# CSMaus/DefectDetection_viaObjectDetection

Measured on AMD Instinct MI355X. Metric: images/sec @640x640 b32 YOLOv8s-seg, higher is better.
Workload: dtype fp16

## Files before the change

defectdetection_viaobjectdetection_amd/_capi.py:

```python
from __future__ import annotations

import ctypes as C
import os

_HERE = os.path.dirname(os.path.abspath(__file__))
LIB_PATH = os.path.join(_HERE, "lib", "libmi355yolo.so")


class M355Error(RuntimeError):
    """Raised when a libmi355yolo call returns a negative status."""


class ModelDesc(C.Structure):
    _fields_ = [("scale", C.c_int), ("nc", C.c_int), ("in_h", C.c_int), ("in_w", C.c_int),
                ("max_batch", C.c_int)]


class ConvInfo(C.Structure):
    _fields_ = [("name", C.c_char * 64), ("cin", C.c_int), ("cout", C.c_int), ("k", C.c_int),
                ("stride", C.c_int), ("has_bn", C.c_int), ("transposed", C.c_int), ("act", C.c_int),
                ("groups", C.c_int)]


class OpInfo(C.Structure):
# ... 44 lines not shown


class LetterboxImage(C.Structure):
    _fields_ = [("offset", C.c_int64), ("h", C.c_int32), ("w", C.c_int32), ("uh", C.c_int32), ("uw", C.c_int32),
                ("top", C.c_int32), ("left", C.c_int32)]


_P = C.c_void_p
_F = C.POINTER(C.c_float)
SIGNATURES = {
    "m355_version": (C.c_char_p, []),
    "m355_last_error": (C.c_char_p, [_P]),
    "m355_create": (C.c_int, [C.POINTER(ModelDesc), C.POINTER(_P)]),
    "m355_destroy": (None, [_P]),
    "m355_num_convs": (C.c_int, [_P]),
    "m355_get_conv_info": (C.c_int, [_P, C.c_int, C.POINTER(ConvInfo)]),
    "m355_num_anchors": (C.c_int, [_P]),
    "m355_pred_width": (C.c_int, [_P]),
    "m355_proto_hw": (C.c_int, [_P, C.POINTER(C.c_int), C.POINTER(C.c_int)]),
    "m355_workspace_bytes": (C.c_size_t, [_P]),
    "m355_flops_per_image": (C.c_double, [_P]),
    "m355_set_conv_weights": (C.c_int, [_P, C.c_int, _P, _P]),
    "m355_forward": (C.c_int, [_P, _P, C.c_int, _P, _P, _P]),
    "m355_num_ops": (C.c_int, [_P]),
    "m355_get_op_info": (C.c_int, [_P, C.c_int, C.POINTER(OpInfo)]),
    "m355_set_profiling": (C.c_int, [_P, C.c_int]),
    "m355_collect_op_times": (C.c_int, [_P, C.POINTER(C.c_double), C.POINTER(C.c_long)]),
    "m355_get_raw_head": (C.c_int, [_P, C.POINTER(_P), C.POINTER(C.c_int)]),
    "m355_copy_raw_head": (C.c_int, [_P, C.c_int, _P, _P]),
    "m355_set_keep_raw": (C.c_int, [_P, C.c_int]),
    "m355_postprocess": (C.c_int, [_P, _P, _P, C.c_int, C.c_float, C.c_float, C.c_int, _P, _P, _P, _P]),
    "m355_conv2d_fwd": (C.c_int, [_P, C.c_int, C.c_int, C.c_int, C.c_int, _P, _P, C.c_int, C.c_int, C.c_int,
                                  C.c_int, _P, _P, C.c_int, C.c_int, _P]),
    "m355_c2f_c32_fwd": (C.c_int, [_P, C.c_int, C.c_int, C.c_int, _P, _P, _P, _P, _P, _P, C.c_int, _P, _P]),
    "m355_bneck_pair_fwd": (C.c_int, [_P, C.c_int, C.c_int, C.c_int, C.c_int, C.c_int, _P, _P, _P, _P, C.c_int, _P, C.c_int, _P]),
    "m355_s2c64_cv1_fwd": (C.c_int, [_P, C.c_int, C.c_int, C.c_int, _P, _P, _P, _P, _P, _P]),
    "m355_stem_s2c32_cv1_fwd": (C.c_int, [_P, C.c_int, C.c_int, C.c_int, _P, _P, _P, _P, _P, _P, _P, C.c_int, _P]),
    "m355_proto_phase_fwd": (C.c_int, [_P, C.c_int, C.c_int, C.c_int, _P, _P, _P, _P, _P, _P, _P, _P]),
    "m355_head_tail_fwd": (C.c_int, [_P, C.c_int, C.c_int, C.c_int, C.c_int, C.c_float, _P, _P, _P, _P, _P, _P, _P, C.c_int, C.c_int, _P]),
    "m355_tal_assign_launch": (C.c_int, [_P, _P, _P, _P, _P, _P, C.c_int32, C.c_int32, C.c_int32, C.c_int32, _P, _P, _P, _P, _P, _P]),
    "m355_conv2d_dgrad": (C.c_int, [_P, C.c_int, C.c_int, C.c_int, C.c_int, _P, C.c_int, C.c_int, C.c_int, _P, _P]),
    "m355_conv2d_wgrad": (C.c_int, [_P, _P, C.c_int, C.c_int, C.c_int, C.c_int, C.c_int, C.c_int, C.c_int, _P, _P]),
    "m355_bn_silu_train_fwd": (C.c_int, [_P, C.c_int, C.c_int, C.c_int, C.c_int, _P, _P, C.c_float, C.c_int, _P, _P, _P, _P, _P]),
    "m355_bn_silu_train_bwd": (C.c_int, [_P, _P, C.c_int, C.c_int, C.c_int, C.c_int, _P, _P, _P, _P, C.c_int, _P, _P, _P, _P]),
    "m355_bn_workspace_floats": (C.c_size_t, [C.c_int]),
    "m355_wgrad_workspace_bytes": (C.c_size_t, [C.c_int32, C.c_int32, C.c_int32, C.c_int32, C.c_int32, C.c_int32]),
    "m355_grad_sumsq_workspace_floats": (C.c_size_t, []),
    "m355_convt2x2_fwd": (C.c_int, [_P, C.c_int, C.c_int, C.c_int, C.c_int, _P, _P, C.c_int, _P, _P]),
    "m355_stem_fwd": (C.c_int, [_P, C.c_int, C.c_int, C.c_int, _P, _P, C.c_int, _P, _P]),
    "m355_stem6_fwd": (C.c_int, [_P, C.c_int, C.c_int, C.c_int, _P, _P, C.c_int, _P, _P]),
    "m355_dwconv3x3_fwd": (C.c_int, [_P, C.c_int, C.c_int, C.c_int, C.c_int, C.c_int, _P, _P, C.c_int, _P, C.c_int, _P]),
    "m355_psa_attn_fwd": (C.c_int, [_P, C.c_int, C.c_int, C.c_int, C.c_int, C.c_int, C.c_int, _P, _P, _P, _P]),
    "m355_sppf_pool": (C.c_int, [_P, C.c_int, C.c_int, C.c_int, C.c_int, _P, _P]),
    "m355_upsample2x": (C.c_int, [_P, C.c_int, C.c_int, C.c_int, C.c_int, _P, _P]),
    "m355_head_decode": (C.c_int, [_P, C.c_int, C.c_int, C.c_int, C.c_int, _P, _P]),
    "m355_nms": (C.c_int, [_P, C.c_int, C.c_int, C.c_int, C.c_int, C.c_float, C.c_float, C.c_int, _P, _P, _P]),
    "m355_conv_launch": (C.c_int, [C.POINTER(ConvLaunchArgs), _P]),
    "m355_wgrad_launch": (C.c_int, [C.POINTER(WgradLaunchArgs), _P]),
    "m355_bn_train_fwd_launch": (C.c_int, [_P, C.c_int64, C.c_int32, C.c_int32, _P, _P, C.c_float, C.c_int32, _P, C.c_int32,
                                           _P, C.c_int32, _P, _P, _P, _P, _P, C.c_float, _P]),
    "m355_bn_train_bwd_launch": (C.c_int, [_P, _P, C.c_int64, C.c_int32, C.c_int32, C.c_int32, _P, _P, _P, _P, C.c_int32,
                                           _P, C.c_int32, _P, _P, _P]),
    "m355_adamw_step": (C.c_int, [_P, _P, _P, _P, _P, _P, C.c_int64, C.c_float, C.c_float, C.c_float, C.c_float, C.c_float,
                                  C.c_float, C.c_int32, C.c_float, C.c_float, _P]),
    "m355_sgd_step": (C.c_int, [_P, _P, _P, _P, _P, C.c_int64, C.c_float, C.c_float, C.c_float, C.c_int32, C.c_float,
                                C.c_float, C.c_float, _P]),
# ... 71 lines not shown
```

defectdetection_viaobjectdetection_amd/csrc/conv1x1_wreg.hip:

```cpp
#include <stdio.h>
#include <stdlib.h>

#include <type_traits>

#include "common.h"

namespace m355 {
namespace {

typedef float float16v __attribute__((ext_vector_type(16)));
constexpr int NWAVES = 8;

__device__ __forceinline__ void dma16(__amdgpu_buffer_rsrc_t rsrc, int voff, int soff, char* lds) {
  __builtin_amdgcn_raw_ptr_buffer_load_lds(rsrc, (__attribute__((address_space(3))) void*)lds, 16, voff, soff, 0, 0);
}
__device__ __forceinline__ int row_plain(int rho) { return 16 * ((rho >> 2) & 1) + 4 * (rho >> 3) + (rho & 3); }

__device__ __forceinline__ void silu16(float16v& v) {
#pragma clang fp contract(off)
  float16v t;
#pragma unroll
  for (int j = 0; j < 16; ++j) t[j] = v[j] * -1.4426950408889634f;
#pragma unroll
  for (int j = 0; j < 16; ++j) t[j] = __builtin_amdgcn_exp2f(t[j]);
// ... 215 lines not shown
    }
    vb += nwg;
    ct = nct; p0 = np0;
    nct = nnct; np0 = nnp0;
    have1 = have2;
    if (ct != ct_cur) {
      load_weights(ct);
      __builtin_amdgcn_s_waitcnt(0x0070);
      __builtin_amdgcn_s_barrier();
    }
  }
}

template <int K, int CB, int PB = 2, bool SPLIT = false>
int launch_w1(const ConvArgs& a, hipStream_t s) {
  using C = W1<K, CB, PB>;
  const int ntiles_px = (a.M + C::TP - 1) / C::TP, ctiles = a.Cout / (CB * 32);
  const int ntiles = ntiles_px * ctiles;
  static int slots = 0;
  auto k = conv1x1_wreg_kernel<K, CB, PB, SPLIT>;
  if (!slots) {
    hipError_t e = hipFuncSetAttribute((const void*)k, hipFuncAttributeMaxDynamicSharedMemorySize, C::LDS_BYTES);
    if (e != hipSuccess) return (int)e;
    int dev = 0, cus = 0;
    if (hipGetDevice(&dev) != hipSuccess || hipDeviceGetAttribute(&cus, hipDeviceAttributeMultiprocessorCount, dev) != hipSuccess)
      return -2;
    slots = cus < 8 ? 8 : cus;
  }
  const int grid = ntiles <= slots ? ntiles : slots;
  hipLaunchKernelGGL(k, dim3(grid), dim3(64 * NWAVES), C::LDS_BYTES, s, a, ntiles_px, ntiles);
  return (int)hipGetLastError();
}

}

bool conv1x1_wreg_ok(const ConvArgs& a) {
  if (a.ksize != 1 || a.stride != 1 || a.pad != 0 || a.out_f32 || a.convt_co > 0 || a.tmode || a.phase || a.w2 || a.dec_preds ||
      a.res)
    return false;
  if (a.Cin != 128 && a.Cin != 192 && a.Cin != 256 && a.Cin != 384 && a.Cin != 512) return false;
  if (a.Cout % 128 || a.Cout > 512 || a.ldx % 8 || a.ldy % 8 || a.Kpad < a.Cin || a.Kpad % 8) return false;
  if (a.Ho != a.Hi || a.Wo != a.Wi) return false;
  if (a.x_bstride != (long)a.Hi * a.Wi * a.ldx || a.y_bstride != (long)a.Ho * a.Wo * a.ldy) return false;
  const int cb = a.Cout % 256 == 0 ? 8 : 4;
  if (cb == 4 && a.Cin > 384) return false;
  if (a.csplit > 0) {
    if (!(a.Cin == 384 && cb == 4) || !a.x2 || a.csplit != 256 || a.ldx2 % 8 || a.x2_bstride % 8 || (a.Hi & 1) ||
        (a.Wi & 1) || a.M >= (1 << 24) || a.M % ((long)a.Ho * a.Wo))
      return false;
    if ((a.M / ((long)a.Ho * a.Wo)) * a.x2_bstride * 2 >= (1L << 31)) return false;
  }
  return (long)a.M * a.ldx * 2 < (1L << 31) && (long)a.M * a.ldy < (1L << 31);
}

int launch_conv1x1_wreg(const ConvArgs& a, hipStream_t s) {
  if (!conv1x1_wreg_ok(a) || !conv_rows_covered(a, 128)) return -1;
  const bool c8 = a.Cout % 256 == 0;
  if (a.csplit > 0 && !(a.Cin == 384 && !c8)) return -1;
  switch (a.Cin) {
    case 128: return c8 ? launch_w1<128, 8>(a, s) : launch_w1<128, 4>(a, s);
    case 192: return c8 ? launch_w1<192, 8>(a, s) : launch_w1<192, 4>(a, s);
    case 256: return c8 ? launch_w1<256, 8>(a, s) : launch_w1<256, 4>(a, s);
    case 384: return c8 ? launch_w1<384, 8>(a, s) : (a.csplit > 0 ? launch_w1<384, 4, 1, true>(a, s) : launch_w1<384, 4, 1, false>(a, s));
    case 512: return c8 ? launch_w1<512, 8>(a, s) : -1;
  }
  return -1;
}

}
```

defectdetection_viaobjectdetection_amd/csrc/engine.hip:

```cpp
#include <math.h>
#include <stdio.h>
#include <stdlib.h>
#include <string.h>

#include <string>
#include <vector>

#include "../../include/mi355yolo.h"
#include "common.h"
#include "engine_types.h"
#include "switches.h"
#include "weight_pack.h"

using namespace m355;

thread_local std::string m355::g_err;

namespace {

void fuse_conv_cv1(m355_engine* e) {
  if (e->sw.no_cvfuse) return;
  for (size_t i = 0; i < e->ops.size(); ++i) {
    Op& oi = e->ops[i];
    if (oi.kind != OP_CONV || oi.out_ext != 0 || oi.res.t >= 0 || oi.in2.t >= 0) continue;
// ... 260 lines not shown
  const PhysConv& p = e->phys[op.conv];
  const Tensor& ti = e->tensors[op.in.t];
  HeadTailArgs a{};
  a.x = ti.p; a.ldx = ti.C; a.M = (long)B * ti.H * ti.W; a.HW = ti.H * ti.W; a.W = ti.W;
  a.stride = (float)(e->desc.in_h / ti.H);
  a.A = e->A; a.level_off = op.level_off; a.nc = e->nc; a.nm = e->nm;
  a.wf = p.wf; a.bias = p.bias; a.preds = preds;
  return a;
}

bool head_tail_layout(const m355_engine* e, const PhysConv& p) {
  return p.diag && p.logical.size() == 3 && p.cin == 224 && p.cout == 64 + e->nc + e->nm && e->nm == 32 && e->nc <= 32 &&
         e->convs[p.logical[0]].cin == 64 && e->convs[p.logical[1]].cin == 128;
}

void plan_route(m355_engine* e, Op& op, const ConvArgs& a) {
  const PlanSwitches& sw = e->sw;
  PhysConv& p = e->phys[op.conv];
  const Tensor& ti = e->tensors[op.in.t];
  if (op.kind == OP_PHASE) {
    op.tile = p.cout % 128 == 0 ? TILE_128x128 : TILE_64x128;
    if (p.l3 >= 0 && p.cin == 128 && p.cout == 128 && p.cout2 == 32 && ti.H % 8 == 0 && ti.W % 16 == 0 && !sw.no_protor)
      op.route = R_PROTOR;
    return;
  }
  const bool conv = op.kind == OP_CONV;
  op.tile = conv_pick_tile(a.Cout, a.M);
  if (a.ksize == 1 && op.tile == TILE_128x128 && sw.k1_tile >= 0) op.tile = sw.k1_tile;
  if (op.decode) op.tile = TILE_128x128;
  if (conv && conv3x3_halo_ok(a) && !sw.no_halo) op.route = R_HALO;
  const bool m32 = op.route == R_HALO && conv3x3_halo_pick(a, proc_switches().no_wide, proc_switches().no_m32) == TILE_M32;
  if (conv && conv3x3_c32_ok(a) && !sw.no_c32) op.route = R_C32;
  if (conv && op.out_ext == 0 && p.l3 < 0 && !p.diag && op.res.t < 0 && !op.decode && (op.in2.t < 0 || !sw.no_w1_split) &&
      conv1x1_wreg_ok(a) && !sw.no_w1)
    op.route = R_W1;
  if (conv && op.route != R_HALO && op.route != R_C32 && conv3x3_slab_ok(a) && !sw.no_slab) op.route = R_SLAB;
  const bool planes_s2 = p.k == 3 && p.stride == 2 && op.res.t < 0 && op.in2.t < 0 && !sw.no_planes_s2;
  const bool planes_m64 = m32 && a.Cout <= 64 && op.res.t < 0 && op.in2.t < 0 && !sw.no_planes_m64;
  if (conv && (op.route == R_SLAB || planes_s2 || planes_m64) && op.out_ext == 0 && p.l3 < 0 && !p.diag && !sw.no_planes) {
    PlanesArgs pa = planes_args(e, op, e->desc.max_batch, 0);
    pa.wfb = (const half_t*)1;
    if (conv3x3_planes_ok(pa)) {
      op.route = R_PLANES;
      p.planes = 1;
    }
  }
  if (conv && op.out_ext == 1 && !op.decode && head_tail_layout(e, p) && ti.C == 224 && op.in.off == 0 && op.raw_off == 0 &&
      a.Ho * a.Wo >= 32 && !sw.no_headtail) {
    op.headtail = 1;
    ++e->headtail_n;
  }
  if (conv && p.l3 >= 0 && p.k == 3 && p.stride == 2 && p.cin == 32 && p.cout == 64 && p.cout2 == 64 && a.Ho % 8 == 0 &&
      a.Wo % 16 == 0 && !sw.no_s2c32)
    op.route = R_S2C32;
  if (conv && p.l3 >= 0 && p.k == 3 && p.stride == 2 && p.cin == 64 && p.cout == 128 && p.cout2 == 128 && a.Ho % 8 == 0 &&
      a.Wo % 8 == 0 && !sw.no_s2c64)
    op.route = R_S2C64;
}

void conv_label(const m355_engine* e, Op& op, const ConvArgs& a) {
  static const char* tile_names[] = {"128x128", "64x128", "32x256", "64x256"};
  const PhysConv& p = e->phys[op.conv];
  char* k = op.kernel;
  const size_t n = sizeof(op.kernel);
  const char* ch = a.Cout > 64 ? "128ch" : "64ch";
  switch (op.route) {
    case R_IGEMM:
// ... 695 lines not shown
```

defectdetection_viaobjectdetection_amd/csrc/op_entries.hip:

```cpp
#include <math.h>
#include <stdio.h>
#include <stdlib.h>

#include <string>
#include <vector>

#include "../../include/mi355yolo.h"
#include "common.h"
#include "switches.h"
#include "weight_pack.h"

using namespace m355;

namespace {

int set_err(int code, const std::string& m) {
  g_err = m;
  return code;
}

struct DevBuf {
  std::vector<void*> p;
  ~DevBuf() { for (void* q : p) (void)hipFree(q); }
  void* alloc(size_t bytes) {
// ... 110 lines not shown
  if (force_tile >= 0 && (force_tile & 0xff) == TILE_PLANES) {
    PlanesArgs pa{};
    pa.x = a.x; pa.x_bstride = a.x_bstride; pa.ldx = a.ldx; pa.H = H; pa.W = W; pa.B = B; pa.Cin = cin; pa.Cout = cout; pa.stride = stride;
    pa.wfb = d.put(planes_frag_pack_padded(rows.data(), cout, Kpad, cin)); pa.cblocks_b = planes_cblocks(cout); pa.bb = a.bias;
    pa.y = (half_t*)d_y; pa.y_bstride = a.y_bstride; pa.ldy = a.ldy;
    pa.res = a.res; pa.r_bstride = a.r_bstride; pa.ldr = a.ldr; pa.act = act; pa.stamps = a.stamps;
    if (!pa.wfb) return alloc_failed();
    char what[80];
    snprintf(what, sizeof(what), "conv3x3_planes B=%d %dx%d %d->%d", B, H, W, cin, cout);
    rc = diag.reps(conv3x3_planes_ok(pa) ? launch_conv3x3_planes(pa, s) : -1, s, what, [&] { return launch_conv3x3_planes(pa, s); });
  } else
  for (int rep = 0; rep < (a.dbg ? 5 : 1); ++rep)
    rc = (force_tile >= 0 && (force_tile & 0xff) == TILE_W1) ? launch_conv1x1_wreg(a, s)
         : (force_tile >= 0 && (force_tile & 0xff) == TILE_C32)
             ? launch_conv3x3_c32(a, s)
             : ((force_tile >= 0 && (force_tile & 0xff) >= TILE_HALO) ? launch_conv3x3_halo(a, (force_tile & 0xff) - TILE_HALO, s)
                                                                       : launch_conv_igemm(a, force_tile, s));
  const hipError_t se = hipStreamSynchronize(s);
  diag.dump(se == hipSuccess);
  return launch_status(rc, se, "conv");
}

}

extern "C" {

int m355_conv2d_fwd(const void* d_x, int B, int H, int W, int cin, const float* h_w, const float* h_bias, int cout,
                    int k, int stride, int act, const void* d_res, void* d_y, int out_f32, int force_tile,
                    void* stream) {
  return conv_op_common(d_x, B, H, W, cin, h_w, h_bias, cout, k, stride, act, d_res, d_y, out_f32, force_tile, 0,
                        stream);
}

int m355_c2f_c32_fwd(const void* d_x, int B, int H, int W, const float* h_wa, const float* h_ba, const float* h_wb,
                     const float* h_bb, const float* h_wc, const float* h_bc, int shortcut, void* d_y, void* stream) {
  if (!d_x || !d_y || !h_wa || !h_ba || !h_wb || !h_bb || !h_wc || !h_bc) return set_err(M355_ERR_INVALID, "null pointer");
  if (B <= 0 || H <= 0 || W <= 0 || H % 8 || W % 16) return set_err(M355_ERR_INVALID, "H must be a multiple of 8 and W of 16");
  hipStream_t s = (hipStream_t)stream;
  const int kp3 = conv_kpad(32, 3), kp1 = conv_kpad(96, 1);
  std::vector<half_t> ra((size_t)32 * kp3, (half_t)0.f), rb((size_t)32 * kp3, (half_t)0.f), rc_((size_t)64 * kp1, (half_t)0.f);
  pack_conv_rows(h_wa, 32, 32, 3, kp3, 0, ra);
  pack_conv_rows(h_wb, 32, 32, 3, kp3, 0, rb);
  pack_conv_rows(h_wc, 64, 96, 1, kp1, 0, rc_);
  std::vector<float> bias(128);
  for (int i = 0; i < 32; ++i) { bias[i] = h_ba[i]; bias[32 + i] = h_bb[i]; }
  for (int i = 0; i < 64; ++i) bias[64 + i] = h_bc[i];
  const FragList fl = frag_list(3, 32, 32);
  DevBuf d;
  const float* db = d.put(bias);
  C2fC32Args a{};
  a.x = (const half_t*)d_x; a.x_bstride = (long)H * W * 64; a.ldx = 64; a.H = H; a.W = W; a.B = B;
  a.wa = d.put(ra); a.wb = d.put(rb); a.wc = d.put(rc_); a.kpad_a = kp3; a.kpad_b = kp3; a.kpad_c = kp1;
  a.waf = d.put(frag_pack(ra.data(), kp3, fl, false)); a.wbf = d.put(frag_pack(rb.data(), kp3, fl, true));
  if (!db || !a.wa || !a.wb || !a.wc || !a.waf || !a.wbf) return alloc_failed();
  a.ba = db; a.bb = db + 32; a.bc = db + 64;
  a.y = (half_t*)d_y; a.y_bstride = (long)H * W * 64; a.ldy = 64; a.shortcut = shortcut;
  const int rc = launch_c2f_c32(a, s);
  return launch_status(rc, hipStreamSynchronize(s), "c2f_c32");
}

int m355_bneck_pair_fwd(const void* d_x, int B, int H, int W, int C, int ldx, const float* h_wa, const float* h_ba, const float* h_wb,
                        const float* h_bb, int shortcut, void* d_y, int ldy, void* stream) {
  if (!d_x || !d_y || !h_wa || !h_ba || !h_wb || !h_bb) return set_err(M355_ERR_INVALID, "null pointer");
  if (B <= 0 || H <= 0 || W <= 0 || C <= 0 || ldx < C || ldy < C) return set_err(M355_ERR_INVALID, "bad shape");
  hipStream_t s = (hipStream_t)stream;
  if (C % 32) return set_err(M355_ERR_INVALID, "C must be a multiple of 32");
// ... 382 lines not shown
                     int mw, int in_h, int in_w, uint8_t* d_masks, void* stream) {
  if (!d_dets || !d_counts || !d_protos || !d_masks) return set_err(M355_ERR_INVALID, "null pointer");
  const int rc = launch_proto_masks(d_dets, d_counts, (const half_t*)d_protos, B, max_det, 32, mh, mw, in_h, in_w,
                                    d_masks, (hipStream_t)stream);
  return rc == 0 ? M355_OK : set_err(M355_ERR_HIP, "mask launch failed: " + std::to_string(rc));
}

int m355_conv_launch(const m355_conv_args* c, void* stream) {
  if (!c || !c->x || !c->w_packed || !c->bias || !c->y || !c->zero_page) return set_err(M355_ERR_INVALID, "null pointer");
  ConvArgs a{};
  a.x = (const half_t*)c->x; a.x_bstride = c->x_bstride; a.ldx = c->ldx; a.Hi = c->hi; a.Wi = c->wi; a.Cin = c->cin;
  a.w = (const half_t*)c->w_packed; a.Kpad = c->kpad; a.bias = c->bias;
  a.y = c->y; a.y_bstride = c->y_bstride; a.ldy = c->ldy; a.Ho = c->ho; a.Wo = c->wo; a.Cout = c->cout;
  a.res = (const half_t*)c->res; a.r_bstride = c->r_bstride; a.ldr = c->ldr;
  a.ksize = c->ksize; a.stride = c->stride; a.pad = c->pad; a.M = c->batch * c->ho * c->wo;
  a.act = c->act; a.out_f32 = c->out_f32; a.convt_co = c->convt_co; a.tmode = c->tmode;
  a.zero = (const half_t*)c->zero_page;
  if (c->convt_co > 0 && c->tmode == 0 && c->ksize == 1 && c->res)
    return set_err(M355_ERR_INVALID, "ConvTranspose (convt_co > 0, ksize 1) takes no residual");
  if (c->tmode == 2) {
    a.tmode = 0;
    a.phase = dgrad_phase_form(c->convt_co, c->cin, c->res != nullptr);
    if (!a.phase)
      return set_err(M355_ERR_INVALID, "tmode 2 needs convt_co % 64 == 0, or 128 % convt_co == 0 with convt_co >= 16 and no res "
                                       "(use the tmode 1 gather)");
  }
  int rc;
  const bool train_w1 = !proc_switches().no_train_w1;
  const bool train_c32 = !proc_switches().no_train_c32;
  if (a.phase == 2 && dgrad_s2c32_ok(a))
    rc = launch_dgrad_s2c32(a, (hipStream_t)stream);
  else if (!a.tmode && conv3x3_halo_ok(a))
    rc = launch_conv3x3_halo(a, 0, (hipStream_t)stream);
  else if (train_w1 && !a.tmode && conv1x1_wreg_ok(a))
    rc = launch_conv1x1_wreg(a, (hipStream_t)stream);
  else if (train_c32 && !a.tmode && conv3x3_c32_ok(a) && conv_rows_covered(a, 32))
    rc = launch_conv3x3_c32(a, (hipStream_t)stream);
  else
    rc = launch_conv_igemm(a, TILE_AUTO, (hipStream_t)stream);
  return rc == 0 ? M355_OK : set_err(M355_ERR_HIP, "conv launch failed: " + std::to_string(rc));
}

int m355_wgrad_launch(const m355_wgrad_args* w, void* stream) {
  if (!w || !w->dz || !w->x || !w->dw || !w->zero_page) return set_err(M355_ERR_INVALID, "null pointer");
  const int rc = launch_conv_wgrad((const half_t*)w->dz, w->dz_bstride, w->lddz, (const half_t*)w->x, w->x_bstride, w->ldx,
                                   w->batch, w->hi, w->wi, w->cin, w->ho, w->wo, w->cout, w->ksize, w->stride, w->pad,
                                   w->dw, (const half_t*)w->zero_page, w->ws, (size_t)(w->ws_bytes < 0 ? 0 : w->ws_bytes),
                                   (hipStream_t)stream);
  if (rc == -3) return set_err(M355_ERR_INVALID, "wgrad workspace missing or smaller than m355_wgrad_workspace_bytes()");
  return rc == 0 ? M355_OK : set_err(M355_ERR_HIP, "wgrad launch failed: " + std::to_string(rc));
}

int m355_bn_train_fwd_launch(const void* z, int64_t npix, int32_t ldz, int32_t C, const float* gamma, const float* beta,
                             float eps, int32_t act, void* y, int32_t ldy, const void* res, int32_t ldr, float* mean,
                             float* invstd, float* ws, float* running_mean, float* running_var, float momentum,
                             void* stream) {
  if (!z || !gamma || !beta || !y || !mean || !invstd || !ws) return set_err(M355_ERR_INVALID, "null pointer");
  const int rc = launch_bn_silu_train_fwd((const half_t*)z, npix, ldz, C, gamma, beta, eps, (half_t*)y, ldy,
                                          (const half_t*)res, ldr, ws, mean, invstd, act, running_mean, running_var, momentum,
                                          (hipStream_t)stream);
  return rc == 0 ? M355_OK : set_err(M355_ERR_HIP, "bn fwd launch failed: " + std::to_string(rc));
}

int m355_bn_train_bwd_launch(const void* z, const void* dy, int64_t npix, int32_t ldz, int32_t lddy, int32_t C,
                             const float* mean, const float* invstd, const float* gamma, const float* beta, int32_t act,
                             void* dz, int32_t lddz, float* dbeta_dgamma, float* ws, void* stream) {
  if (!z || !dy || !mean || !invstd || !gamma || !beta || !dz || !dbeta_dgamma || !ws) return set_err(M355_ERR_INVALID, "null pointer");
// ... 211 lines not shown
```

defectdetection_viaobjectdetection_amd/csrc/switches.h:

```cpp
#pragma once

namespace m355 {

struct ProcSwitches {
  bool no_fast_epi, no_wide, no_m32, no_bias_lds, static_tiles, no_persist, stem_gather;
  int persist, halo_variant, smallm;
  bool c2f_noprio;
  const char* c2f_stamps;
  int c32_waste, c32_slots, m32_slots, wide_slots, wide_stagger;
  int s2c32_dbg, s2c32_ring, s2c64_prio, protor_prio;
  const char *s2c32_stamps, *s2c64_stamps, *protor_stamps;
  int stem2_nxb;
  bool no_stemfuse;
  int sppf_minblocks, mask_dbg, mask_tile;
  bool no_dgrad_s2c32, no_wgrad_stem, no_wgrad_s2c32, no_wgrad3, no_train_w1, no_train_c32;
  int wgrad_blocks, w2_blocks_x2, wgrad3_shrink, wgrad3_blocks, wgrad3_mintiles;
  long wgrad3_slabmb;
};
const ProcSwitches& proc_switches();

struct PlanSwitches {
  bool no_c2f32, no_pair, no_protofuse, no_protofuse3, no_upfuse;
  int lane_plan[4];
  bool no_cvfuse, decfuse, no_lanes, no_subbatch;
  bool no_stemfuse;
  int subbatch, subbatch_ops;
  bool no_protor, no_halo, no_c32, no_w1_split, no_w1, no_slab, no_planes_s2, no_planes_m64, no_planes, no_headtail, no_s2c32,
      no_s2c64;
  int k1_tile;
  long headtail_maxm;
};
PlanSwitches read_plan_switches();

bool live_no_stem2();
bool live_no_dgrad_phases();
bool live_pair64();
const char* live_stamps_path();
int live_bneck_reps();

}
```

defectdetection_viaobjectdetection_amd/csrc/switches.hip:

```cpp
#include "switches.h"

#include <limits.h>
#include <stdlib.h>

namespace m355 {

namespace {

bool env_set(const char* name) { return getenv(name) != nullptr; }
long env_int(const char* name, long unset) {
  const char* v = getenv(name);
  return v ? atol(v) : unset;
}

ProcSwitches read_proc_switches() {
  ProcSwitches v{};
  v.no_fast_epi = env_set("M355_NO_FAST_EPI");
  v.no_wide = env_set("M355_NO_WIDE");
  v.no_m32 = env_set("M355_NO_M32");
  v.no_bias_lds = env_set("M355_NO_BIAS_LDS");
  v.static_tiles = env_set("M355_STATIC_TILES");
  v.no_persist = env_set("M355_NO_PERSIST");
  v.stem_gather = env_set("M355_STEM_GATHER");
  v.persist = env_int("M355_PERSIST", 0);
// ... 34 lines not shown
}

}

const ProcSwitches& proc_switches() {
  static const ProcSwitches v = read_proc_switches();
  return v;
}

PlanSwitches read_plan_switches() {
  PlanSwitches v{};
  v.no_c2f32 = env_set("M355_NO_C2F32");
  v.no_pair = env_set("M355_NO_PAIR");
  v.no_protofuse = env_set("M355_NO_PROTOFUSE");
  v.no_protofuse3 = env_set("M355_NO_PROTOFUSE3");
  v.no_upfuse = env_set("M355_NO_UPFUSE");
  const int lanes[4] = {1, 2, 2, 0};
  const char* lp = getenv("M355_LANE_PLAN");
  for (int i = 0; i < 4; ++i) {
    if (lp && (lp[i] < '0' || lp[i] > '3')) lp = nullptr;
    v.lane_plan[i] = lp ? lp[i] - '0' : lanes[i];
  }
  v.no_cvfuse = env_set("M355_NO_CVFUSE");
  v.decfuse = env_set("M355_DECFUSE");
  v.no_lanes = env_set("M355_NO_LANES");
  v.no_subbatch = env_set("M355_NO_SUBBATCH");
  v.no_stemfuse = env_set("M355_NO_STEMFUSE");
  v.subbatch = env_int("M355_SUBBATCH", 0);
  v.subbatch_ops = env_int("M355_SUBBATCH_OPS", INT_MAX);
  v.no_protor = env_set("M355_NO_PROTOR");
  v.no_halo = env_set("M355_NO_HALO");
  v.no_c32 = env_set("M355_NO_C32");
  v.no_w1_split = env_set("M355_NO_W1_SPLIT");
  v.no_w1 = env_set("M355_NO_W1");
  v.no_slab = env_set("M355_NO_SLAB");
  v.no_planes_s2 = env_set("M355_NO_PLANES_S2");
  v.no_planes_m64 = env_set("M355_NO_PLANES_M64");
  v.no_planes = env_set("M355_NO_PLANES");
  v.no_headtail = env_set("M355_NO_HEADTAIL");
  v.no_s2c32 = env_set("M355_NO_S2C32");
  v.no_s2c64 = env_set("M355_NO_S2C64");
  v.k1_tile = env_int("M355_K1_TILE", -1);
  v.headtail_maxm = env_int("M355_HEADTAIL_MAXM", 0);
  return v;
}

bool live_no_stem2() { return env_set("M355_NO_STEM2"); }
bool live_no_dgrad_phases() { return env_set("M355_NO_DGRAD_PHASES"); }
bool live_pair64() { return env_set("M355_PAIR64"); }
const char* live_stamps_path() { return getenv("M355_STAMPS"); }
int live_bneck_reps() { return env_int("M355_BNECK_REPS", 0); }

}
```

defectdetection_viaobjectdetection_amd/csrc/weight_pack.hip:

```cpp
#include "weight_pack.h"

#include <algorithm>

namespace m355 {

void pack_conv_rows(const float* w, int cout, int cin, int k, int Kpad, int row0, std::vector<half_t>& dst, int koff) {
  for (int co = 0; co < cout; ++co)
    for (int ci = 0; ci < cin; ++ci)
      for (int kh = 0; kh < k; ++kh)
        for (int kw = 0; kw < k; ++kw)
          dst[(size_t)(row0 + co) * Kpad + koff + (kh * k + kw) * cin + ci] =
              (half_t)w[(((size_t)co * cin + ci) * k + kh) * k + kw];
}

void pack_convt2x2_rows(const float* w, int cin, int cout, int Kpad, std::vector<half_t>& dst) {
  for (int c = 0; c < cin; ++c)
    for (int co = 0; co < cout; ++co)
      for (int dy = 0; dy < 2; ++dy)
        for (int dx = 0; dx < 2; ++dx)
          dst[(size_t)((dy * 2 + dx) * cout + co) * Kpad + c] = (half_t)w[(((size_t)c * cout + co) * 2 + dy) * 2 + dx];
}

std::vector<half_t> pack_stem3x3(const float* w, int cout) {
  std::vector<half_t> sw((size_t)cout * 32, (half_t)0.f);
// ... 4 lines not shown
  return sw;
}

std::vector<half_t> to_half_vec(const float* w, size_t n) {
  std::vector<half_t> r(n);
  for (size_t i = 0; i < n; ++i) r[i] = (half_t)w[i];
  return r;
}

static int frag_row(int rho, bool operand) {
  if (!operand) return 16 * ((rho >> 2) & 1) + 4 * (rho >> 3) + (rho & 3);
  const int q = rho >> 3, h = (rho >> 2) & 1, i = rho & 3;
  return 16 * (q >> 1) + 8 * h + 4 * (q & 1) + i;
}
std::vector<half_t> frag_pack(const half_t* rows, int Kpad, const FragList& frags, bool operand) {
  std::vector<half_t> out(frags.size() * 512);
  for (size_t f = 0; f < frags.size(); ++f)
    for (int lane = 0; lane < 64; ++lane) {
      const half_t* src = rows + (size_t)(frags[f].first + frag_row(lane & 31, operand)) * Kpad + frags[f].second + 8 * (lane >> 5);
      for (int j = 0; j < 8; ++j) out[(f * 64 + lane) * 8 + j] = src[j];
    }
  return out;
}
FragList frag_grid(int rows, int K) {
  FragList f;
  for (int r = 0; r < rows; r += 32)
    for (int k = 0; k < K; k += 16) f.push_back({r, k});
  return f;
}

FragList frag_list(int k, int cin, int cout) {
  const bool taken = (k == 3 && cin == 64 && cout == 128) ||
                     (k == 3 && cin == 32 && (cout == 64 || cout == 32)) ||
                     (k == 1 && (cin == 128 || cin == 192 || cin == 256 || cin == 384 || cin == 512) && cout % 128 == 0 && cout <= 512);
  return taken ? frag_grid(cout, k * k * cin) : FragList();
}

FragList head_level_frags(int nc) {
  FragList f = frag_grid(64, 64);
  for (int sl = 0; sl < 8; ++sl) f.push_back({64, 64 + 16 * sl});
  for (int sl = 0; sl < 2; ++sl) f.push_back({64 + nc, 192 + 16 * sl});
  return f;
}

FragList epilogue_frags(int cout2, int k) { return frag_grid(cout2, k); }

void compose_proto_phases(int n, const float* wtp, const float* btp, const float* w3p, const float* b3p, int cout_pad, int Kpad,
                          std::vector<half_t>& rows, std::vector<float>& btab) {
    rows.assign((size_t)cout_pad * Kpad, (half_t)0.f);
    std::vector<double> acc((size_t)n * n);
    for (int py = 0; py < 2; ++py)
      for (int px = 0; px < 2; ++px)
        for (int aa = 0; aa < 2; ++aa)
          for (int bb = 0; bb < 2; ++bb) {
            std::fill(acc.begin(), acc.end(), 0.0);
            for (int kh = 0; kh < 3; ++kh) {
              const int ty = py + kh - 1, ry = (ty < 0 ? -1 : ty / 2), dy = ty & 1;
              if (ry + 1 - py != aa) continue;
              for (int kw = 0; kw < 3; ++kw) {
                const int tx = px + kw - 1, rx = (tx < 0 ? -1 : tx / 2), dx = tx & 1;
                if (rx + 1 - px != bb) continue;
                for (int co = 0; co < n; ++co)
                  for (int c = 0; c < n; ++c) {
                    const double w3 = w3p[(((size_t)co * n + c) * 3 + kh) * 3 + kw];
                    if (w3 == 0.0) continue;
                    const float* wt = wtp;
                    double* ar = &acc[(size_t)co * n];
// ... 43 lines not shown
```

include/mi355yolo.h:

```cpp
#ifndef MI355YOLO_H_
#define MI355YOLO_H_

#include <stddef.h>
#include <stdint.h>

#ifdef __cplusplus
extern "C" {
#endif

typedef struct m355_engine m355_engine;

typedef enum {
  M355_OK = 0,
  M355_ERR_INVALID = -1,
  M355_ERR_NO_DEVICE = -2,
  M355_ERR_HIP = -3,
  M355_ERR_STATE = -4,
  M355_ERR_NOMEM = -5
} m355_status;

typedef struct {
  int scale;
  int nc;
  int in_h, in_w;
// ... 28 lines not shown
int m355_set_conv_weights(m355_engine* e, int idx, const float* w, const float* bias);

int m355_forward(m355_engine* e, const void* d_in_u8_nhwc, int batch, float* d_preds, void* d_protos,
                 void* stream);

typedef struct {
  char kernel[48];
  char layer[64];
  double flops_per_image;
  double bytes_per_image;
  double weight_bytes;
} m355_op_info;
int m355_num_ops(const m355_engine* e);
int m355_get_op_info(const m355_engine* e, int idx, m355_op_info* out);
int m355_set_profiling(m355_engine* e, int enable);
int m355_collect_op_times(m355_engine* e, double* ms_sum, long* counts);

int m355_get_raw_head(m355_engine* e, const float** d_raw, int* width);
int m355_copy_raw_head(m355_engine* e, int batch, float* d_out, void* stream);
int m355_set_keep_raw(m355_engine* e, int keep);

int m355_postprocess(m355_engine* e, const float* d_preds, const void* d_protos, int batch, float conf,
                     float iou, int max_det, float* d_dets, int* d_counts, uint8_t* d_masks, void* stream);
int m355_postprocess_ex(m355_engine* e, const float* d_preds, const void* d_protos, int batch, float conf, float iou,
                        int max_det, int agnostic, const uint32_t* d_class_mask, float* d_dets, int* d_counts,
                        uint8_t* d_masks, void* stream);



int m355_conv2d_fwd(const void* d_x_f16_nhwc, int B, int H, int W, int cin, const float* h_w,
                    const float* h_bias, int cout, int k, int stride, int act,
                    const void* d_res_f16_nhwc, void* d_y_f16_nhwc, int out_f32, int force_tile,
                    void* stream);
int m355_c2f_c32_fwd(const void* d_x_f16_nhwc, int B, int H, int W, const float* h_wa, const float* h_ba,
                     const float* h_wb, const float* h_bb, const float* h_wc, const float* h_bc, int shortcut,
                     void* d_y_f16_nhwc, void* stream);
int m355_bneck_pair_fwd(const void* d_x_f16_nhwc, int B, int H, int W, int C, int ldx, const float* h_wa, const float* h_ba,
                        const float* h_wb, const float* h_bb, int shortcut, void* d_y_f16_nhwc, int ldy, void* stream);
int m355_s2c64_cv1_fwd(const void* d_x_f16_nhwc, int B, int H, int W, const float* h_w3, const float* h_b3, const float* h_w1,
                       const float* h_b1, void* d_y_f16_nhwc, void* stream);
int m355_stem_s2c32_cv1_fwd(const void* d_in_u8_nhwc, int B, int H, int W, const float* h_w0, const float* h_b0, const float* h_w1,
                            const float* h_b1, const float* h_w2, const float* h_b2, void* d_y_f16_nhwc, int two_team, void* stream);
int m355_proto_phase_fwd(const void* d_x_f16_nhwc, int B, int H, int W, const float* h_wt, const float* h_bt, const float* h_w3,
                         const float* h_b3, const float* h_wc, const float* h_bc, void* d_y_f16_nhwc, void* stream);
int m355_head_tail_fwd(const void* d_x_f16_nhwc, int B, int H, int W, int nc, float stride, const float* h_w2, const float* h_b2,
                       const float* h_w3, const float* h_b3, const float* h_w4, const float* h_b4, float* d_preds, int A, int level_off,
                       void* stream);
int m355_conv2d_dgrad(const void* d_dy_f16_nhwc, int B, int H, int W, int cin, const float* h_w, int cout, int k,
                      int stride, void* d_dx_f16_nhwc, void* stream);
int m355_conv2d_wgrad(const void* d_x_f16_nhwc, const void* d_dy_f16_nhwc, int B, int H, int W, int cin, int cout,
                      int k, int stride, float* d_dw_krsc, void* stream);
size_t m355_bn_workspace_floats(int C);
int m355_bn_silu_train_fwd(const void* d_z, int B, int H, int W, int C, const float* d_gamma, const float* d_beta,
                           float eps, int act, void* d_y, float* d_mean, float* d_invstd, float* d_ws, void* stream);
int m355_bn_silu_train_bwd(const void* d_z, const void* d_dy, int B, int H, int W, int C, const float* d_mean,
                           const float* d_invstd, const float* d_gamma, const float* d_beta, int act, void* d_dz,
                           float* d_dbeta_dgamma, float* d_ws, void* stream);
int m355_convt2x2_fwd(const void* d_x_f16_nhwc, int B, int H, int W, int cin, const float* h_w,
                      const float* h_bias, int cout, void* d_y_f16_nhwc, void* stream);
int m355_stem_fwd(const void* d_in_u8, int B, int H, int W, const float* h_w, const float* h_bias, int cout,
                  void* d_y_f16_nhwc, void* stream);
int m355_stem6_fwd(const void* d_x_u8_nhwc, int B, int H, int W, const float* h_w, const float* h_bias, int C0,
                   void* d_y_f16_nhwc, void* stream);
int m355_dwconv3x3_fwd(const void* d_x_f16_nhwc, int B, int H, int W, int C, int ldx, const float* h_w, const float* h_b,
                       int act, void* d_y_f16_nhwc, int ldy, void* stream);
int m355_psa_attn_fwd(const void* d_qkv_f16_nhwc, int B, int H, int W, int heads, int key_dim, int head_dim,
// ... 171 lines not shown
```

Measured before the change: 18160.

## Add deep-K 1x1 conv kernel for Cin 768/1024 with weight-register streaming

Adds a new 1x1 convolution kernel for Cin of 768 and 1024 with Cout a multiple of 256. It streams activation tiles into an 8-stage LDS ring through buffer-to-LDS DMA and double-buffers weight chunks in registers, one 128-channel K chunk at a time. It also supports the concat-split input form, where the upsampled operand is read at half resolution from a second tensor. The engine routes these layers (for example the SPPF and neck C2f cv2 convs) to the new kernel by default; an env switch disables it, and training keeps the old path. A standalone conv_op test entry point is added as well.

```diff
diff --git a/defectdetection_viaobjectdetection_amd/_capi.py b/defectdetection_viaobjectdetection_amd/_capi.py
--- a/defectdetection_viaobjectdetection_amd/_capi.py
+++ b/defectdetection_viaobjectdetection_amd/_capi.py
@@ -100,6 +100,8 @@
     "m355_postprocess": (C.c_int, [_P, _P, _P, C.c_int, C.c_float, C.c_float, C.c_int, _P, _P, _P, _P]),
     "m355_conv2d_fwd": (C.c_int, [_P, C.c_int, C.c_int, C.c_int, C.c_int, _P, _P, C.c_int, C.c_int, C.c_int,
                                   C.c_int, _P, _P, C.c_int, C.c_int, _P]),
+    "m355_conv_op": (C.c_int, [_P, C.c_int, _P, C.c_int, C.c_int, C.c_int, C.c_int, C.c_int, C.c_int, _P, _P, C.c_int, C.c_int, _P,
+                               C.c_int, C.c_int, _P]),
     "m355_c2f_c32_fwd": (C.c_int, [_P, C.c_int, C.c_int, C.c_int, _P, _P, _P, _P, _P, _P, C.c_int, _P, _P]),
     "m355_bneck_pair_fwd": (C.c_int, [_P, C.c_int, C.c_int, C.c_int, C.c_int, C.c_int, _P, _P, _P, _P, C.c_int, _P, C.c_int, _P]),
     "m355_s2c64_cv1_fwd": (C.c_int, [_P, C.c_int, C.c_int, C.c_int, _P, _P, _P, _P, _P, _P]),
diff --git a/defectdetection_viaobjectdetection_amd/csrc/conv1x1_wreg.hip b/defectdetection_viaobjectdetection_amd/csrc/conv1x1_wreg.hip
--- a/defectdetection_viaobjectdetection_amd/csrc/conv1x1_wreg.hip
+++ b/defectdetection_viaobjectdetection_amd/csrc/conv1x1_wreg.hip
@@ -271,21 +271,211 @@
   return (int)hipGetLastError();
 }
 
+template <int K>
+struct WD {
+  static constexpr int KC = 128;
+  static constexpr int NC = K / KC;
+  static constexpr int KS = K / 16;
+  static constexpr int SP = 64;
+  static constexpr int STAGE_BYTES = SP * KC * 2;
+  static constexpr int NST = 8;
+  static constexpr int AHEAD = 7;
+  static constexpr int P_IT = STAGE_BYTES / 1024 / NWAVES;
+  static constexpr int STG_OFF = NST * STAGE_BYTES;
+  static constexpr int LDS_BYTES = STG_OFF + NWAVES * 2048;
+  static_assert(K % 256 == 0 && NC % 2 == 0 && P_IT == 2 && LDS_BYTES <= 160 * 1024, "shape");
+};
+
+template <int K, bool SPLIT>
+__global__ __launch_bounds__(512, 1) void conv1x1_wreg_deepk_kernel(const ConvArgs a, int ngran, int nb) {
+  using C = WD<K>;
+  extern __shared__ __attribute__((aligned(16))) char smem[];
+  const int tid = threadIdx.x, lane = tid & 63;
+  const int wave = __builtin_amdgcn_readfirstlane(tid >> 6);
+  const int n = lane & 31, h = lane >> 5;
+  const int ct = blockIdx.x / nb, bi = blockIdx.x - ct * nb;
+  const int P0 = 32 * (int)((long)bi * ngran / nb), P1 = 32 * (int)((long)(bi + 1) * ngran / nb);
+  if (P0 >= P1) return;
+  const int pend = P1 < a.M ? P1 : a.M;
+
+  const __amdgpu_buffer_rsrc_t rs_x = __builtin_amdgcn_make_buffer_rsrc((void*)a.x, 0, (int)((long)a.M * a.ldx * 2), 0x00020000);
+  const int HW = a.Ho * a.Wo;
+  const __amdgpu_buffer_rsrc_t rs_x2 = __builtin_amdgcn_make_buffer_rsrc(
+      (void*)(SPLIT ? a.x2 : a.x), 0, SPLIT ? (int)((long)(a.M / HW) * a.x2_bstride * 2) : 0, 0x00020000);
+  const float inv_hw = 1.0f / (float)HW, inv_w = 1.0f / (float)a.Wo;
+  const int nsplit = SPLIT ? a.csplit / C::KC : 0;
+
+  const int ngr = (P1 - P0) >> 5;
+  const int total = C::NC * (2 * (ngr >> 2) + (((ngr & 3) + 1) >> 1));
+  int ipst = P0, ic = 0, it = 0, iq = 0;
+  auto issue_next = [&]() __attribute__((always_inline)) {
+    if (iq >= total) return;
+    const int pb0 = ipst + C::SP * it;
+    const int npx = pend - pb0;
+    int ln;
+    asm volatile("v_mbcnt_lo_u32_b32 %0, -1, 0\n\tv_mbcnt_hi_u32_b32 %0, -1, %0" : "=v"(ln));
+    char* const sb = smem + (iq & (C::NST - 1)) * C::STAGE_BYTES;
+#pragma unroll
+    for (int i = 0; i < C::P_IT; ++i) {
+      const int g = wave + NWAVES * i;
+      const int cid = 64 * g + ln, px = cid >> 4, slot = cid & 15;
+      const int cc = (slot ^ px) & 15;
+      if (SPLIT && ic < nsplit) {
+        int b, pix, ho, wo;
+        fdivmod(pb0 + (px < npx ? px : 0), HW, inv_hw, b, pix);
+        fdivmod(pix, a.Wo, inv_w, ho, wo);
+        dma16(rs_x2, px < npx ? (int)(((long)b * a.x2_bstride + ((long)(ho >> 1) * (a.Wo >> 1) + (wo >> 1)) * a.ldx2 + ic * C::KC + cc * 8) * 2)
+                              : (int)0x80000000, 0, sb + g * 1024);
+      } else {
+        dma16(rs_x, px < npx ? (px * a.ldx + ic * C::KC + cc * 8) * 2 : (int)0x80000000, pb0 * a.ldx * 2, sb + g * 1024);
+      }
+    }
+    ++iq;
+    const int rem = (P1 - ipst) >> 5;
+    if (++it == (rem > 2 ? 2 : 1)) {
+      it = 0;
+      if (++ic == C::NC) { ic = 0; ipst += 128; }
+    }
+  };
+  const __amdgpu_buffer_rsrc_t rs_w = a.wf
+      ? __builtin_amdgcn_make_buffer_rsrc((void*)(a.wf + (long)(ct * 8 + wave) * C::KS * 512), 0, C::KS * 1024, 0x00020000)
+      : __builtin_amdgcn_make_buffer_rsrc((void*)(a.w + (long)(ct * 256 + 32 * wave) * a.Kpad), 0, 32 * a.Kpad * 2, 0x00020000);
+  const int w_voff = a.wf ? lane * 16 : (row_plain(n) * a.Kpad + 8 * h) * 2;
+  const int w_sl = a.wf ? 1024 : 32;
+  half8 wv[2][8];
+  auto load_weights = [&](int set, int c) __attribute__((always_inline)) {
+#pragma unroll
+    for (int s = 0; s < 8; ++s)
+      wv[set][s] = __builtin_bit_cast(half8, __builtin_amdgcn_raw_buffer_load_b128(rs_w, w_voff, (c * 8 + s) * w_sl, 0));
+  };
+
+  load_weights(0, 0);
+#pragma unroll
+  for (int i = 0; i < C::AHEAD; ++i) issue_next();
+  float16v bv;
+  {
+    const float* bp = a.bias + ct * 256 + 32 * wave + 16 * h;
+#pragma unroll
+    for (int j = 0; j < 16; ++j) bv[j] = bp[j];
+  }
+
+  const int rkey = h ^ (n & 15);
+  char* const stg = smem + C::STG_OFF + wave * 2048;
+  const int st_p = lane >> 2, st_k = lane & 3;
+  int q = 0;
+  for (int pst = P0; pst < P1; pst += 128) {
+    const int npb = (P1 - pst) >> 5 < 4 ? (P1 - pst) >> 5 : 4;
+    float16v acc[4];
+#pragma unroll
+    for (int pb = 0; pb < 4; ++pb) acc[pb] = bv;
+#pragma unroll
+    for (int c = 0; c < C::NC; ++c) {
+#pragma unroll
+      for (int t = 0; t < 2; ++t) {
+        if (t == 0 || npb > 2) {
+          if (total - 1 - q >= C::AHEAD - 1) __builtin_amdgcn_s_waitcnt(0x0070 | (2 * (C::AHEAD - 1)));
+          else __builtin_amdgcn_s_waitcnt(0x0070);
+          __builtin_amdgcn_s_barrier();
+          issue_next();
+          if (t == 0) {
+            if (c + 1 < C::NC) load_weights((c + 1) & 1, c + 1);
+            else if (pst + 128 < P1) load_weights(0, 0);
+          }
+          const char* const xb = smem + (q & (C::NST - 1)) * C::STAGE_BYTES + n * 256;
+          auto stage = [&](auto npbs) __attribute__((always_inline)) {
+            constexpr int PBS = decltype(npbs)::value;
+            half8 fr[2][PBS][2];
+            auto read_group = [&](int g) __attribute__((always_inline)) {
+#pragma unroll
+              for (int s = 0; s < 2; ++s)
+#pragma unroll
+                for (int pbs = 0; pbs < PBS; ++pbs)
+                  fr[g & 1][pbs][s] = *(const half8*)(xb + pbs * 32 * 256 + (((2 * (2 * g + s)) ^ rkey) << 4));
+            };
+            read_group(0);
+            __builtin_amdgcn_sched_barrier(0);
+#pragma unroll
+            for (int g = 0; g < 4; ++g) {
+              if (g + 1 < 4) read_group(g + 1);
+#pragma unroll
+              for (int s = 0; s < 2; ++s)
+#pragma unroll
+                for (int pbs = 0; pbs < PBS; ++pbs)
+                  acc[2 * t + pbs] = __builtin_amdgcn_mfma_f32_32x32x16_f16(wv[c & 1][2 * g + s], fr[g & 1][pbs][s], acc[2 * t + pbs], 0, 0, 0);
+              __builtin_amdgcn_sched_barrier(0);
+            }
+          };
+          if (2 * t + 1 < npb) stage(std::integral_constant<int, 2>{});
+          else stage(std::integral_constant<int, 1>{});
+          ++q;
+        }
+      }
+    }
+    {
+      half_t* const yb = (half_t*)a.y + (long)pst * a.ldy + ct * 256 + 32 * wave;
+#pragma unroll
+      for (int pb = 0; pb < 4; ++pb) {
+        if (pb < npb) {
+          if (a.act) silu16(acc[pb]);
+          half8 o0, o1;
+#pragma unroll
+          for (int j = 0; j < 8; ++j) {
+            o0[j] = m355_to_half(acc[pb][j]);
+            o1[j] = m355_to_half(acc[pb][8 + j]);
+          }
+          asm volatile("s_waitcnt lgkmcnt(0)" ::: "memory");
+          *(half8*)(stg + n * 64 + (((2 * h) ^ ((n >> 1) & 3)) << 4)) = o0;
+          *(half8*)(stg + n * 64 + (((2 * h + 1) ^ ((n >> 1) & 3)) << 4)) = o1;
+          asm volatile("s_waitcnt lgkmcnt(0)" ::: "memory");
+#pragma unroll
+          for (int i = 0; i < 2; ++i) {
+            const int p = 16 * i + st_p;
+            const half8 v = *(const half8*)(stg + p * 64 + ((st_k ^ ((p >> 1) & 3)) << 4));
+            if (pst + 32 * pb + p < a.M) *(half8*)(yb + (long)(32 * pb + p) * a.ldy + st_k * 8) = v;
+          }
+        }
+      }
+    }
+  }
+}
+
+template <int K, bool SPLIT>
+int launch_wd(const ConvArgs& a, hipStream_t s) {
+  using C = WD<K>;
+  static int slots = 0;
+  auto k = conv1x1_wreg_deepk_kernel<K, SPLIT>;
+  if (!slots) {
+    hipError_t e = hipFuncSetAttribute((const void*)k, hipFuncAttributeMaxDynamicSharedMemorySize, C::LDS_BYTES);
+    if (e != hipSuccess) return (int)e;
+    int dev = 0, cus = 0;
+    if (hipGetDevice(&dev) != hipSuccess || hipDeviceGetAttribute(&cus, hipDeviceAttributeMultiprocessorCount, dev) != hipSuccess)
+      return -2;
+    slots = cus < 8 ? 8 : cus;
+  }
+  const int ngran = (a.M + 31) / 32, ctiles = a.Cout / 256;
+  int nb = slots / ctiles;
+  if (nb > ngran) nb = ngran;
+  hipLaunchKernelGGL(k, dim3(nb * ctiles), dim3(64 * NWAVES), C::LDS_BYTES, s, a, ngran, nb);
+  return (int)hipGetLastError();
+}
+
 }
 
 bool conv1x1_wreg_ok(const ConvArgs& a) {
   if (a.ksize != 1 || a.stride != 1 || a.pad != 0 || a.out_f32 || a.convt_co > 0 || a.tmode || a.phase || a.w2 || a.dec_preds ||
       a.res)
     return false;
-  if (a.Cin != 128 && a.Cin != 192 && a.Cin != 256 && a.Cin != 384 && a.Cin != 512) return false;
+  const bool deep = a.Cin == 768 || a.Cin == 1024;
+  if (a.Cin != 128 && a.Cin != 192 && a.Cin != 256 && a.Cin != 384 && a.Cin != 512 && !deep) return false;
   if (a.Cout % 128 || a.Cout > 512 || a.ldx % 8 || a.ldy % 8 || a.Kpad < a.Cin || a.Kpad % 8) return false;
   if (a.Ho != a.Hi || a.Wo != a.Wi) return false;
   if (a.x_bstride != (long)a.Hi * a.Wi * a.ldx || a.y_bstride != (long)a.Ho * a.Wo * a.ldy) return false;
   const int cb = a.Cout % 256 == 0 ? 8 : 4;
   if (cb == 4 && a.Cin > 384) return false;
   if (a.csplit > 0) {
-    if (!(a.Cin == 384 && cb == 4) || !a.x2 || a.csplit != 256 || a.ldx2 % 8 || a.x2_bstride % 8 || (a.Hi & 1) ||
-        (a.Wi & 1) || a.M >= (1 << 24) || a.M % ((long)a.Ho * a.Wo))
+    const bool form = (a.Cin == 384 && cb == 4 && a.csplit == 256) || (a.Cin == 768 && a.csplit == 512);
+    if (!form || !a.x2 || a.ldx2 % 8 || a.x2_bstride % 8 || (a.Hi & 1) || (a.Wi & 1) || a.M >= (1 << 24) ||
+        a.M % ((long)a.Ho * a.Wo))
       return false;
     if ((a.M / ((long)a.Ho * a.Wo)) * a.x2_bstride * 2 >= (1L << 31)) return false;
   }
@@ -295,8 +485,10 @@
 int launch_conv1x1_wreg(const ConvArgs& a, hipStream_t s) {
   if (!conv1x1_wreg_ok(a) || !conv_rows_covered(a, 128)) return -1;
   const bool c8 = a.Cout % 256 == 0;
-  if (a.csplit > 0 && !(a.Cin == 384 && !c8)) return -1;
+  if (a.csplit > 0 && !(a.Cin == 384 && !c8) && a.Cin != 768) return -1;
   switch (a.Cin) {
+    case 768: return !c8 ? -1 : a.csplit > 0 ? launch_wd<768, true>(a, s) : launch_wd<768, false>(a, s);
+    case 1024: return c8 ? launch_wd<1024, false>(a, s) : -1;
     case 128: return c8 ? launch_w1<128, 8>(a, s) : launch_w1<128, 4>(a, s);
     case 192: return c8 ? launch_w1<192, 8>(a, s) : launch_w1<192, 4>(a, s);
     case 256: return c8 ? launch_w1<256, 8>(a, s) : launch_w1<256, 4>(a, s);
diff --git a/defectdetection_viaobjectdetection_amd/csrc/engine.hip b/defectdetection_viaobjectdetection_amd/csrc/engine.hip
--- a/defectdetection_viaobjectdetection_amd/csrc/engine.hip
+++ b/defectdetection_viaobjectdetection_amd/csrc/engine.hip
@@ -316,7 +316,7 @@
   const bool m32 = op.route == R_HALO && conv3x3_halo_pick(a, proc_switches().no_wide, proc_switches().no_m32) == TILE_M32;
   if (conv && conv3x3_c32_ok(a) && !sw.no_c32) op.route = R_C32;
   if (conv && op.out_ext == 0 && p.l3 < 0 && !p.diag && op.res.t < 0 && !op.decode && (op.in2.t < 0 || !sw.no_w1_split) &&
-      conv1x1_wreg_ok(a) && !sw.no_w1)
+      (p.cin <= 512 || !sw.no_w1_deepk) && conv1x1_wreg_ok(a) && !sw.no_w1)
     op.route = R_W1;
   if (conv && op.route != R_HALO && op.route != R_C32 && conv3x3_slab_ok(a) && !sw.no_slab) op.route = R_SLAB;
   const bool planes_s2 = p.k == 3 && p.stride == 2 && op.res.t < 0 && op.in2.t < 0 && !sw.no_planes_s2;
diff --git a/defectdetection_viaobjectdetection_amd/csrc/op_entries.hip b/defectdetection_viaobjectdetection_amd/csrc/op_entries.hip
--- a/defectdetection_viaobjectdetection_amd/csrc/op_entries.hip
+++ b/defectdetection_viaobjectdetection_amd/csrc/op_entries.hip
@@ -166,6 +166,37 @@
                         stream);
 }
 
+int m355_conv_op(const void* d_x, int ldx, const void* d_x2, int ldx2, int csplit, int B, int H, int W, int cin, const float* h_w,
+                 const float* h_bias, int cout, int act, void* d_y, int ldy, int force_tile, void* stream) {
+  if (!d_x || !h_w || !h_bias || !d_y || (csplit > 0 && !d_x2)) return set_err(M355_ERR_INVALID, "null pointer");
+  if (cin <= 0 || cout <= 0 || B <= 0 || H <= 0 || W <= 0 || ldx < cin - csplit || ldy < cout || csplit < 0 || csplit >= cin ||
+      (csplit > 0 && (ldx2 < csplit || (H & 1) || (W & 1))))
+    return set_err(M355_ERR_INVALID, "bad shape");
+  hipStream_t s = (hipStream_t)stream;
+  const int tile = force_tile >= 0 ? (force_tile & 0xff) : TILE_AUTO;
+  const int cout_pad = conv_cout_pad(cout), Kpad = conv_kpad(cin, 1);
+  int bch = 0;
+  if (tile >= 0 && (tile == TILE_PLANES || tile == TILE_C32 || tile >= TILE_HALO && tile != TILE_W1 || !conv_forced_tile_extent(tile, cout, &bch, nullptr) ||
+                    (cout + bch - 1) / bch * bch > cout_pad))
+    return set_err(M355_ERR_INVALID, "forced tile " + std::to_string(tile) + " is not a 1x1 kernel's, or reads past the packed weight rows");
+  std::vector<half_t> rows((size_t)cout_pad * Kpad, (half_t)0.f);
+  std::vector<float> bias(cout_pad, 0.f);
+  pack_conv_rows(h_w, cout, cin, 1, Kpad, 0, rows);
+  for (int i = 0; i < cout; ++i) bias[i] = h_bias[i];
+  const FragList fl = frag_list(1, cin, cout);
+  DevBuf d;
+  ConvArgs a{};
+  a.x = (const half_t*)d_x; a.x_bstride = (long)H * W * ldx; a.ldx = ldx; a.Hi = H; a.Wi = W; a.Cin = cin;
+  a.w = d.put(rows); a.Kpad = Kpad; a.bias = d.put(bias); a.zero = (const half_t*)d.zeroed(256); a.act = act;
+  a.w_rows = cout_pad; a.wf = fl.empty() ? nullptr : d.put(frag_pack(rows.data(), Kpad, fl, false));
+  if (!a.w || !a.bias || !a.zero || (!fl.empty() && !a.wf)) return alloc_failed();
+  a.y = d_y; a.ksize = 1; a.stride = 1; a.pad = 0; a.Ho = H; a.Wo = W; a.Cout = cout;
+  a.y_bstride = (long)H * W * ldy; a.ldy = ldy; a.M = B * H * W;
+  if (csplit > 0) { a.x2 = (const half_t*)d_x2; a.ldx2 = ldx2; a.x2_bstride = (long)(H / 2) * (W / 2) * ldx2; a.csplit = csplit; }
+  const int rc = tile == TILE_W1 ? launch_conv1x1_wreg(a, s) : launch_conv_igemm(a, tile, s);
+  return launch_status(rc, hipStreamSynchronize(s), "conv_op");
+}
+
 int m355_c2f_c32_fwd(const void* d_x, int B, int H, int W, const float* h_wa, const float* h_ba, const float* h_wb,
                      const float* h_bb, const float* h_wc, const float* h_bc, int shortcut, void* d_y, void* stream) {
   if (!d_x || !d_y || !h_wa || !h_ba || !h_wb || !h_bb || !h_wc || !h_bc) return set_err(M355_ERR_INVALID, "null pointer");
@@ -614,7 +645,7 @@
     rc = launch_dgrad_s2c32(a, (hipStream_t)stream);
   else if (!a.tmode && conv3x3_halo_ok(a))
     rc = launch_conv3x3_halo(a, 0, (hipStream_t)stream);
-  else if (train_w1 && !a.tmode && conv1x1_wreg_ok(a))
+  else if (train_w1 && !a.tmode && a.Cin <= 512 && conv1x1_wreg_ok(a))
     rc = launch_conv1x1_wreg(a, (hipStream_t)stream);
   else if (train_c32 && !a.tmode && conv3x3_c32_ok(a) && conv_rows_covered(a, 32))
     rc = launch_conv3x3_c32(a, (hipStream_t)stream);
diff --git a/defectdetection_viaobjectdetection_amd/csrc/switches.h b/defectdetection_viaobjectdetection_amd/csrc/switches.h
--- a/defectdetection_viaobjectdetection_amd/csrc/switches.h
+++ b/defectdetection_viaobjectdetection_amd/csrc/switches.h
@@ -25,7 +25,7 @@
   bool no_cvfuse, decfuse, no_lanes, no_subbatch;
   bool no_stemfuse;
   int subbatch, subbatch_ops;
-  bool no_protor, no_halo, no_c32, no_w1_split, no_w1, no_slab, no_planes_s2, no_planes_m64, no_planes, no_headtail, no_s2c32,
+  bool no_protor, no_halo, no_c32, no_w1_split, no_w1_deepk, no_w1, no_slab, no_planes_s2, no_planes_m64, no_planes, no_headtail, no_s2c32,
       no_s2c64;
   int k1_tile;
   long headtail_maxm;
diff --git a/defectdetection_viaobjectdetection_amd/csrc/switches.hip b/defectdetection_viaobjectdetection_amd/csrc/switches.hip
--- a/defectdetection_viaobjectdetection_amd/csrc/switches.hip
+++ b/defectdetection_viaobjectdetection_amd/csrc/switches.hip
@@ -90,6 +90,7 @@
   v.no_halo = env_set("M355_NO_HALO");
   v.no_c32 = env_set("M355_NO_C32");
   v.no_w1_split = env_set("M355_NO_W1_SPLIT");
+  v.no_w1_deepk = env_set("M355_NO_W1_DEEPK");
   v.no_w1 = env_set("M355_NO_W1");
   v.no_slab = env_set("M355_NO_SLAB");
   v.no_planes_s2 = env_set("M355_NO_PLANES_S2");
diff --git a/defectdetection_viaobjectdetection_amd/csrc/weight_pack.hip b/defectdetection_viaobjectdetection_amd/csrc/weight_pack.hip
--- a/defectdetection_viaobjectdetection_amd/csrc/weight_pack.hip
+++ b/defectdetection_viaobjectdetection_amd/csrc/weight_pack.hip
@@ -60,7 +60,8 @@
 FragList frag_list(int k, int cin, int cout) {
   const bool taken = (k == 3 && cin == 64 && cout == 128) ||
                      (k == 3 && cin == 32 && (cout == 64 || cout == 32)) ||
-                     (k == 1 && (cin == 128 || cin == 192 || cin == 256 || cin == 384 || cin == 512) && cout % 128 == 0 && cout <= 512);
+                     (k == 1 && (cin == 128 || cin == 192 || cin == 256 || cin == 384 || cin == 512) && cout % 128 == 0 && cout <= 512) ||
+                     (k == 1 && (cin == 768 || cin == 1024) && cout % 256 == 0 && cout <= 512);
   return taken ? frag_grid(cout, k * k * cin) : FragList();
 }
 
diff --git a/include/mi355yolo.h b/include/mi355yolo.h
--- a/include/mi355yolo.h
+++ b/include/mi355yolo.h
@@ -84,6 +84,8 @@
                     const float* h_bias, int cout, int k, int stride, int act,
                     const void* d_res_f16_nhwc, void* d_y_f16_nhwc, int out_f32, int force_tile,
                     void* stream);
+int m355_conv_op(const void* d_x_f16, int ldx, const void* d_x2_f16, int ldx2, int csplit, int B, int H, int W, int cin,
+                 const float* h_w, const float* h_bias, int cout, int act, void* d_y_f16, int ldy, int force_tile, void* stream);
 int m355_c2f_c32_fwd(const void* d_x_f16_nhwc, int B, int H, int W, const float* h_wa, const float* h_ba,
                      const float* h_wb, const float* h_bb, const float* h_wc, const float* h_bc, int shortcut,
                      void* d_y_f16_nhwc, void* stream);
```

Result: no change. 18020 (-0.8%).
